# randyjhc/vit-colmap

Measured on AMD Instinct MI355X. Metric: images/sec extracted + pair-matches/sec (N×D brute-force NN), higher is better.
Workload: dtype bf16 (ViT) / u8+i32 (matcher); 1 GPU; configs[1]+configs[2]: DINOv2 ViT-S/14 extract of 50 640x480 images (512 keypoints, 384-D uint8 descriptors) then exhaustive mutual-NN + ratio matching of all pairs among the extracted images; images_total=50, images_rank0=50, num_keypoints=512, descriptor_dim=384, parallelism=images+pairs sharded x1

## Files before the change

### include/vitcolmap_hip.h

```cpp
#ifndef VITCOLMAP_HIP_H_
#define VITCOLMAP_HIP_H_

#include <stddef.h>
#include <stdint.h>

#ifdef __cplusplus
extern "C" {
#endif

#define VC_ABI_VERSION 1

#define VC_OK 0
#define VC_ERR_INVALID_ARG (-1)
#define VC_ERR_UNSUPPORTED (-2)
#define VC_ERR_LAUNCH (-3)
#define VC_ERR_WORKSPACE (-4)

#define VC_MAX_KEYPOINTS 2048
#define VC_MAX_DESC_DIM 1024
#define VC_MAX_NEIGHBOURS 64

typedef void* vc_stream_t;

int vc_abi_version(void);
// ... 83 lines not shown
#define VC_METHOD_HARRIS 0
#define VC_METHOD_DOG 1
#define VC_METHOD_COMBINED 2

int vc_structure_tensor(const void* tokens, int token_dtype, int n_images, int H, int W, int C,
                        float* st, vc_stream_t stream);

int vc_score_map(const float* st, int n_images, int H, int W, int method, float* score,
                 vc_stream_t stream);

int vc_select_keypoints(const float* score, int n_images, int H, int W, int target, int bin_size,
                        float nms_radius, int kmax, int32_t* out_yx, float* out_score,
                        int32_t* out_count, int32_t* dbg_cand_yx, float* dbg_cand_score,
                        int32_t* dbg_cand_count, vc_stream_t stream);

int vc_describe(const void* tokens, int token_dtype, int n_images, int H, int W, int C,
                const int32_t* yx, const int32_t* count, int kmax, const float* proj, int dd,
                int resized_w, int resized_h, int orig_w, int orig_h, float* out_kp,
                float* out_desc_f32, uint8_t* out_desc_u8, vc_stream_t stream);

#define VC_NORM_L2 0
#define VC_NORM_ROOTSIFT 1
int vc_describe_at(const void* tokens, int token_dtype, int n_images, int H, int W, int C, const float* keypoints_xy,
                   const int32_t* count, int kmax, const float* proj, int dd, int feat_w, int feat_h, int orig_w,
                   int orig_h, int normalisation, float* out_desc_f32, uint8_t* out_desc_u8, vc_stream_t stream);

int vc_quantize_u8(const float* in, uint8_t* out, size_t n, vc_stream_t stream);

size_t vc_heatmap_workspace_bytes(int n_images, int H, int W, int kmax);
int vc_heatmap_keypoints(const float* kp_map, const float* desc_map, long long desc_image_stride,
// ... 31 lines not shown
int vc_conv_taps_bf16(void* x, const void* weight, const void* bias, void* out, int batch, int height, int width, int c_in,
                      int n_out, int kh, int kw, int dy0, int dx0, int out_parity, int epilogue, vc_stream_t stream);

size_t vc_linear_xs_weight_bytes(int n_out, int k_in);
int vc_linear_xs_prepare(const float* weight, const float* bias_or_null, const float* ln_gamma_or_null,
                         const float* ln_beta_or_null, int n_out, int k_in, void* weight_tiled,
                         float* bias_folded, vc_stream_t stream);
int vc_linear_xs_bf16(const void* x, const void* weight_tiled, const float* bias_folded,
                      const void* residual_or_null, void* out, int rows, int n_out, int k_in, int epilogue,
                      int fuse_layernorm, float ln_eps, const void* gelu_table_or_null, vc_stream_t stream);
size_t vc_gelu_table_bytes(void);
int vc_gelu_table_bf16(void* table, vc_stream_t stream);

int vc_patch_embed_bf16(const void* patches, const void* weight, const void* bias, const void* pos_embed,
                        void* out, int n_images, int tokens, int n_out, int k_in, vc_stream_t stream);

size_t vc_mlp_weight_bytes(int n_hidden, int dim);
int vc_mlp_prepare(const float* w1, const float* b1_or_null, const float* ln_gamma_or_null,
                   const float* ln_beta_or_null, const float* w2, const float* b2_or_null, int n_hidden, int dim,
                   void* weights_tiled, float* b1_folded, float* b2_out, vc_stream_t stream);
int vc_mlp_bf16(void* x_inout, const void* weights_tiled, const float* b1_folded, const float* b2,
                const void* gelu_table, int rows, int n_hidden, int dim, float ln_eps, vc_stream_t stream);

#define VC_SIFT_MAX_RADIUS 64
#define VC_SIFT_NORM_L2 0
#define VC_SIFT_NORM_L1_ROOT 1

int vc_sift_grey(const uint8_t* images_bgr, int n_images, int h, int w, int out_h, int out_w, int upsample, float* out,
                 vc_stream_t stream);
int vc_sift_blur(const float* src, float* tmp, float* dst, int n_images, int h, int w, const float* taps, int radius,
// ... 31 lines not shown
```

### vit_colmap_amd/_lib.py

```python
import ctypes
import os
from ctypes import POINTER, c_char_p, c_double, c_float, c_int, c_int32, c_size_t, c_uint8, c_uint32, c_void_p

_HERE = os.path.dirname(os.path.abspath(__file__))
LIB_PATH = os.environ.get("VITCOLMAP_HIP_LIB") or os.path.join(_HERE, "libvitcolmap_hip.so")

VC_OK = 0
ABI_VERSION = 1
VC_MAX_KEYPOINTS = 2048
VC_MAX_DESC_DIM = 1024
VC_MAX_NEIGHBOURS = 64
VC_BA_MAX_CAMS = 512
VC_ERR_INVALID_ARG, VC_ERR_UNSUPPORTED, VC_ERR_LAUNCH, VC_ERR_WORKSPACE = -1, -2, -3, -4


class HipLibraryError(RuntimeError):
    pass


_u8p, _i32p, _u32p, _f32p = POINTER(c_uint8), POINTER(c_int32), POINTER(c_uint32), POINTER(ctypes.c_float)

SIGNATURES = {
    "vc_abi_version": (c_int, []),
    "vc_status_string": (c_char_p, [c_int]),
# ... 23 lines not shown
    "vc_p3p": (c_int, [c_void_p, c_void_p, c_void_p, c_int, c_void_p, c_int, c_void_p, c_void_p, c_void_p]),
    "vc_absolute_pose_score": (c_int, [c_void_p, c_void_p, c_void_p, c_int, c_void_p, c_int, c_float, c_void_p, c_void_p]),
    "vc_absolute_pose_inliers": (c_int, [c_void_p, c_void_p, c_void_p, c_int, c_void_p, c_float, c_void_p, c_void_p]),
    "vc_triangulate_tracks": (c_int, [c_void_p, c_void_p, c_void_p, c_int, c_void_p, c_int, c_void_p, c_double, c_double, c_void_p,
                                      c_void_p, c_void_p, c_void_p, c_void_p]),
    "vc_ba_linearize_points": (c_int, [c_void_p, c_int, c_void_p, c_void_p, c_int, c_void_p, c_void_p, c_void_p, c_int, c_double,
                                       c_void_p, c_void_p, c_void_p, c_void_p, c_void_p, c_void_p, c_void_p, c_void_p]),
    "vc_ba_reduce_cameras": (c_int, [c_int, c_void_p, c_int, c_void_p, c_void_p, c_int, c_void_p, c_void_p, c_void_p, c_double,
                                     c_void_p, c_void_p, c_void_p, c_void_p, c_void_p, c_void_p, c_void_p]),
    "vc_ba_step": (c_int, [c_void_p, c_int, c_void_p, c_int, c_void_p, c_void_p, c_int, c_void_p, c_void_p, c_void_p, c_void_p,
                           c_void_p, c_void_p, c_void_p, c_void_p, c_void_p]),
    "vc_structure_tensor": (c_int, [c_void_p, c_int, c_int, c_int, c_int, c_int, c_void_p, c_void_p]),
    "vc_score_map": (c_int, [c_void_p, c_int, c_int, c_int, c_int, c_void_p, c_void_p]),
    "vc_select_keypoints": (c_int, [c_void_p, c_int, c_int, c_int, c_int, c_int, c_float, c_int, c_void_p,
                                    c_void_p, c_void_p, c_void_p, c_void_p, c_void_p, c_void_p]),
    "vc_describe": (c_int, [c_void_p, c_int, c_int, c_int, c_int, c_int, c_void_p, c_void_p, c_int, c_void_p,
                            c_int, c_int, c_int, c_int, c_int, c_void_p, c_void_p, c_void_p, c_void_p]),
    "vc_describe_at": (c_int, [c_void_p, c_int, c_int, c_int, c_int, c_int, c_void_p, c_void_p, c_int, c_void_p, c_int, c_int,
                               c_int, c_int, c_int, c_int, c_void_p, c_void_p, c_void_p]),
    "vc_quantize_u8": (c_int, [c_void_p, c_void_p, c_size_t, c_void_p]),
    "vc_heatmap_workspace_bytes": (c_size_t, [c_int, c_int, c_int, c_int]),
    "vc_heatmap_keypoints": (c_int, [c_void_p, c_void_p, ctypes.c_longlong, ctypes.c_longlong, ctypes.c_longlong, c_int, c_int,
                                     c_int, c_int, c_int, c_float, c_int, c_float, c_float, c_float, c_float, c_void_p,
                                     c_void_p, c_void_p, c_void_p, c_void_p]),
    "vc_add_layernorm_bf16": (c_int, [c_void_p, c_void_p, c_void_p, c_void_p, c_float, c_int, c_int, c_void_p,
                                      c_void_p, c_void_p]),
    "vc_layernorm_drop_first_bf16": (c_int, [c_void_p, c_void_p, c_void_p, c_float, c_int, c_int, c_int, c_void_p, c_void_p]),
    "vc_attention_bf16": (c_int, [c_void_p, c_int, c_int, c_int, c_int, c_int, c_void_p, c_void_p]),
    "vc_linear_bf16": (c_int, [c_void_p, c_void_p, c_void_p, c_void_p, c_void_p, c_int, c_int, c_int, c_int, c_void_p]),
    "vc_conv_taps_bf16": (c_int, [c_void_p, c_void_p, c_void_p, c_void_p] + [c_int] * 11 + [c_void_p]),
    "vc_linear_xs_weight_bytes": (c_size_t, [c_int, c_int]),
    "vc_linear_xs_prepare": (c_int, [c_void_p, c_void_p, c_void_p, c_void_p, c_int, c_int, c_void_p, c_void_p, c_void_p]),
    "vc_linear_xs_bf16": (c_int, [c_void_p, c_void_p, c_void_p, c_void_p, c_void_p, c_int, c_int, c_int, c_int, c_int,
                                  c_float, c_void_p, c_void_p]),
    "vc_gelu_table_bytes": (c_size_t, []),
    "vc_gelu_table_bf16": (c_int, [c_void_p, c_void_p]),
    "vc_patch_embed_bf16": (c_int, [c_void_p, c_void_p, c_void_p, c_void_p, c_void_p, c_int, c_int, c_int, c_int, c_void_p]),
    "vc_mlp_weight_bytes": (c_size_t, [c_int, c_int]),
    "vc_mlp_prepare": (c_int, [c_void_p, c_void_p, c_void_p, c_void_p, c_void_p, c_void_p, c_int, c_int, c_void_p, c_void_p,
                               c_void_p, c_void_p]),
    "vc_mlp_bf16": (c_int, [c_void_p, c_void_p, c_void_p, c_void_p, c_void_p, c_int, c_int, c_int, c_float, c_void_p]),
    "vc_preprocess_u8": (c_int, [c_void_p, c_int, c_int, c_int, c_int, c_int, c_int, c_int, c_void_p, c_void_p,
                                 c_void_p]),
    "vc_sift_grey": (c_int, [c_void_p, c_int, c_int, c_int, c_int, c_int, c_int, c_void_p, c_void_p]),
    "vc_sift_blur": (c_int, [c_void_p, c_void_p, c_void_p, c_int, c_int, c_int, _f32p, c_int, c_void_p]),
    "vc_sift_downsample": (c_int, [c_void_p, c_int, c_int, c_int, c_void_p, c_void_p]),
    "vc_sift_dog": (c_int, [c_void_p, c_int, c_int, c_int, c_int, c_void_p, c_void_p]),
    "vc_sift_detect": (c_int, [c_void_p, c_int, c_int, c_int, c_int, c_float, c_float, c_int, c_void_p, c_int, c_void_p,
                               c_void_p, c_void_p]),
    "vc_sift_orient": (c_int, [c_void_p, c_int, c_int, c_int, c_int, c_void_p, c_void_p, c_int, c_int, c_int, c_void_p,
                               c_void_p, c_void_p]),
    "vc_sift_describe": (c_int, [c_void_p, c_int, c_int, c_int, c_int, c_void_p, c_void_p, c_int, c_void_p, c_void_p, c_int,
# ... 92 lines not shown
```

### vit_colmap_amd/csrc/gemm.hip

```cpp
#include <hip/hip_runtime.h>
#include <stdint.h>

#include "../../include/vitcolmap_hip.h"
#include "common.h"
#include "device.h"

namespace {

typedef __bf16 v8bf __attribute__((ext_vector_type(8)));
typedef __bf16 v4bf __attribute__((ext_vector_type(4)));
typedef __bf16 v2bf __attribute__((ext_vector_type(2)));
typedef float v16f __attribute__((ext_vector_type(16)));
typedef float v4f __attribute__((ext_vector_type(4)));
typedef float v2f __attribute__((ext_vector_type(2)));
typedef uint32_t v4u __attribute__((ext_vector_type(4)));
typedef uint32_t v2u __attribute__((ext_vector_type(2)));

__device__ __forceinline__ uint32_t pack_bf16x2(float lo, float hi) {
  const v2bf p = {(__bf16)lo, (__bf16)hi};
  return *(const uint32_t*)&p;
}
__device__ __forceinline__ v2f unpack_bf16x2(uint32_t u) { return (v2f){__uint_as_float(u << 16), __uint_as_float(u & 0xffff0000u)}; }

constexpr int BM = 128;
// ... 39 lines not shown
__device__ __forceinline__ float swiglu_f32(float a, float b) {
  const float e = __builtin_amdgcn_exp2f(a * -1.4426950408889634f);
  return a * __builtin_amdgcn_rcpf(1.0f + e) * b;
}

__device__ __forceinline__ uint32_t frag_off(int row0, int lane, int ks) {
  const int fr = lane & 15, ch = ks * 4 + (lane >> 4);
  return (uint32_t)(row0 + fr) * 128u + (uint32_t)((ch ^ (fr & 7)) << 4);
}

template <int EPI>
__global__ __launch_bounds__(256, 2) void gemm_kernel(const __bf16* __restrict__ X, const __bf16* __restrict__ W,
                                                      const __bf16* __restrict__ bias,
                                                      const __bf16* __restrict__ res, __bf16* __restrict__ out,
                                                      int M, int N, int K, int n_tiles_n, int n_tiles,
                                                      int group) {
  __shared__ __attribute__((aligned(1024))) uint8_t lds[2][kStage];
  const int tid = threadIdx.x, lane = tid & 63;
  const int wave = __builtin_amdgcn_readfirstlane(tid >> 6);
  const int wm = wave & 1, wn = wave >> 1;

  const int tile = vc::xcd_tile(blockIdx.x, n_tiles);
  const int tm = tile / n_tiles_n, tn = tile - tm * n_tiles_n;
  const int m0 = tm * BM, n0 = tn * BN;
  const int H = N >> 1, j0 = tn * (BN / 2);

  const uint32_t lds0 = vc::lds_addr(&lds[0][0]);
  const int prow = lane >> 3, pchunk = (lane & 7) ^ prow;
  const __bf16* xsrc[4];
  const __bf16* wsrc[4];
#pragma unroll
// ... 86 lines not shown
#pragma unroll
        for (int j = 0; j < 4; ++j) v[j] = acc[a][b][j] + (float)bv[j];
        if (EPI == EPI_GELU) {
#pragma unroll
          for (int j = 0; j < 4; ++j) v[j] = gelu_erf(v[j]);
        }
        if (EPI == EPI_RESIDUAL || EPI == EPI_PATCH) {
          const v4bf rv = *(const v4bf*)(res + ro);
#pragma unroll
          for (int j = 0; j < 4; ++j) v[j] += (float)rv[j];
        }
        v4bf ov;
#pragma unroll
        for (int j = 0; j < 4; ++j) ov[j] = (__bf16)v[j];
        *(v4bf*)(out + o) = ov;
      }
    }
  }
}


constexpr int G2M = 256, G2N = 256;
constexpr int kUnit2 = 128 * 128;
constexpr int kBuf2 = 4 * kUnit2;
constexpr int G256_LDS = 2 * kBuf2;
constexpr int kAhead2 = 6;

template <int EPI, bool CONV>
__global__ __launch_bounds__(512, 2) void gemm256_kernel(const __bf16* __restrict__ X, const __bf16* __restrict__ W,
                                                         const __bf16* __restrict__ bias, const __bf16* __restrict__ res,
// ... 887 lines not shown
    static vc::PerDeviceOnce configured;
    if (int st = vc::allow_dynamic_lds(configured, G256_LDS, gemm256_kernel<EPI_BIAS, false>, gemm256_kernel<EPI_GELU, false>,
                                       gemm256_kernel<EPI_RESIDUAL, false>, gemm256_kernel<EPI_SWIGLU, false>))
      return st;
    const dim3 grid(persistent_grid(nt, cus)), block(512);
    return vc::dispatch<EPI_BIAS, EPI_GELU, EPI_RESIDUAL, EPI_SWIGLU>(epilogue, [&](auto epi) {
      hipLaunchKernelGGL((gemm256_kernel<epi, false>), grid, block, (size_t)G256_LDS, s, px, pw, pb, pr, po, rows, n_out, k_in,
                         tiles_n, (int)nt, 0, 0, 0, 1, 0, 0, -1);
      return vc::check_launch();
    });
  }
  const int tiles_m = (rows + BM - 1) / BM, tiles_n = n_out / BN;
  const long long nt = (long long)tiles_m * tiles_n;
  if (nt > 0x7fffffffLL) return VC_ERR_UNSUPPORTED;
  return vc::dispatch<EPI_BIAS, EPI_GELU, EPI_RESIDUAL, EPI_SWIGLU>(epilogue, [&](auto epi) {
    hipLaunchKernelGGL(gemm_kernel<epi>, dim3((unsigned)nt), dim3(256), 0, s, px, pw, pb, pr, po, rows, n_out, k_in, tiles_n, (int)nt, 1);
    return vc::check_launch();
  });
}


int vc_conv_taps_bf16(void* x, const void* weight, const void* bias, void* out, int batch, int height, int width, int c_in,
                      int n_out, int kh, int kw, int dy0, int dx0, int out_parity, int epilogue, vc_stream_t stream) {
  if (!x || !weight || !bias || !out || batch < 0 || height <= 0 || width <= 0 || c_in <= 0 || n_out <= 0) return VC_ERR_INVALID_ARG;
  if (epilogue != EPI_BIAS && epilogue != EPI_GELU) return VC_ERR_INVALID_ARG;
  if (kh <= 0 || kw <= 0 || kh * kw > 16 || dy0 < -8 || dy0 > 8 || dx0 < -8 || dx0 > 8) return VC_ERR_INVALID_ARG;
  if (out_parity < -1 || out_parity > 3) return VC_ERR_INVALID_ARG;
  if (n_out % G2N != 0 || c_in % BK != 0) return VC_ERR_UNSUPPORTED;
  if (!aligned16(x, weight, bias, out)) return VC_ERR_INVALID_ARG;
  const long long rows = (long long)batch * height * width;
  if (rows == 0) return VC_OK;
// ... 72 lines not shown
                         ln_eps, gt);
      return vc::check_launch();
    };
    return vc::dispatch<EPI_BIAS, EPI_GELU, EPI_RESIDUAL>(epilogue, [&](auto epi) {
      return vc::dispatch<true, false>(fuse_layernorm != 0, [&](auto ln) {
        if constexpr (epi == EPI_GELU) {
          if (use_gt) return launch(epi, ln, std::true_type{});
        }
        return launch(epi, ln, std::false_type{});
      });
    });
  });
}


int vc_patch_embed_bf16(const void* patches, const void* weight, const void* bias, const void* pos_embed, void* out,
                        int n_images, int tokens, int n_out, int k_in, vc_stream_t stream) {
  if (!patches || !weight || !bias || !pos_embed || !out || n_images < 0 || tokens <= 0 || n_out <= 0 || k_in <= 0)
    return VC_ERR_INVALID_ARG;
  if (n_out % BN != 0 || k_in % BK != 0) return VC_ERR_UNSUPPORTED;
  if (!aligned16(patches, weight, bias, pos_embed, out)) return VC_ERR_INVALID_ARG;
  if (n_images == 0) return VC_OK;
  const long long rows = (long long)n_images * tokens;
  const long long nt = ((rows + BM - 1) / BM) * (n_out / BN);
  if (rows > 0x7fffffffLL || nt > 0x7fffffffLL) return VC_ERR_UNSUPPORTED;
  hipLaunchKernelGGL(gemm_kernel<EPI_PATCH>, dim3((unsigned)nt), dim3(256), 0, (hipStream_t)stream, (const __bf16*)patches,
                     (const __bf16*)weight, (const __bf16*)bias, (const __bf16*)pos_embed, (__bf16*)out, (int)rows, n_out,
                     k_in, n_out / BN, (int)nt, tokens);
  return vc::check_launch();
}


size_t vc_mlp_weight_bytes(int n_hidden, int dim) {
  if (dim != XK || n_hidden <= 0 || n_hidden % 32 != 0 || n_hidden > mlp_lds().max_hidden()) return 0;
  return (size_t)(n_hidden / 32) * MStage;
}

int vc_mlp_prepare(const float* w1, const float* b1_or_null, const float* ln_gamma_or_null, const float* ln_beta_or_null,
                   const float* w2, const float* b2_or_null, int n_hidden, int dim, void* weights_tiled, float* b1_folded,
                   float* b2_out, vc_stream_t stream) {
  if (!w1 || !w2 || !weights_tiled || !b1_folded || !b2_out) return VC_ERR_INVALID_ARG;
  if (vc_mlp_weight_bytes(n_hidden, dim) == 0) return VC_ERR_UNSUPPORTED;
  if ((ln_gamma_or_null == nullptr) != (ln_beta_or_null == nullptr)) return VC_ERR_INVALID_ARG;
  hipLaunchKernelGGL(mlp_prepare_kernel, dim3((n_hidden + XK + 3) / 4), dim3(256), 0, (hipStream_t)stream, w1, b1_or_null,
// ... 22 lines not shown
```

### vit_colmap_amd/csrc/select.hip

```cpp
#include <hip/hip_runtime.h>
#include <stdint.h>

#include "../../include/vitcolmap_hip.h"
#include "common.h"
#include "device.h"

namespace {

constexpr int kMaxCells = 16384;
constexpr int kMaxCandidates = 4096;
constexpr int kSelThreads = 512;

template <typename T>
__device__ inline float load_token(const T* p, int i);
template <>
__device__ inline float load_token<float>(const float* p, int i) { return p[i]; }
template <>
__device__ inline float load_token<uint16_t>(const uint16_t* p, int i) { return vc::bf16_to_f32(p[i]); }

__device__ inline float wave_sum(float v) {
#pragma unroll
  for (int o = 32; o > 0; o >>= 1) v += __shfl_xor(v, o);
  return v;
}
// ... 111 lines not shown
  if (hi > 0.f)
    for (int i = threadIdx.x; i < cells; i += blockDim.x) m[i] = m[i] / hi;
  __syncthreads();
}

__device__ inline void minmax_eps(float* m, int cells, float* scratch) {
  float lo = INFINITY, hi = -INFINITY;
  for (int i = threadIdx.x; i < cells; i += blockDim.x) { lo = fminf(lo, m[i]); hi = fmaxf(hi, m[i]); }
  lo = block_reduce(lo, false, scratch);
  hi = block_reduce(hi, true, scratch);
  const float den = (hi - lo) + 1e-8f;
  for (int i = threadIdx.x; i < cells; i += blockDim.x) m[i] = (m[i] - lo) / den;
  __syncthreads();
}

__global__ __launch_bounds__(kSelThreads) void score_kernel(const float* __restrict__ st, int H, int W, int method,
                                                            Taps g3, Taps g7, Taps g11, float* __restrict__ score) {
  extern __shared__ __attribute__((aligned(16))) float lds[];
  const int cells = H * W;
  float* a = lds;
  float* b = lds + cells;
  float* scratch = lds + 2 * cells;
  const int img = blockIdx.x;
  const float* ixx = st + (size_t)img * 4 * cells;
  const float* iyy = ixx + cells;
  const float* ixy = iyy + cells;
  const float* avg = ixy + cells;

  if (method == 0 || method == 2) {
    for (int i = threadIdx.x; i < cells; i += blockDim.x) {
      const int y = i / W, x = i - y * W;
      const float sxx = smooth(ixx, H, W, y, x, g3);
      const float syy = smooth(iyy, H, W, y, x, g3);
      const float sxy = smooth(ixy, H, W, y, x, g3);
      const float det = sxx * syy - sxy * sxy;
      const float tr = sxx + syy;
      const float corner = det - 0.04f * (tr * tr);
      const float edge = sqrtf(sxx + syy);
      a[i] = 0.7f * corner + 0.3f * edge;
    }
    __syncthreads();
    minmax01(a, cells, scratch);
  }
  if (method == 1 || method == 2) {
    float* o = method == 1 ? a : b;
    for (int i = threadIdx.x; i < cells; i += blockDim.x) {
      const int y = i / W, x = i - y * W;
      o[i] = fabsf(smooth(avg, H, W, y, x, g7) - smooth(avg, H, W, y, x, g11));
    }
    __syncthreads();
    minmax01(o, cells, scratch);
  }
  if (method == 2) {
    minmax_eps(a, cells, scratch);
    minmax_eps(b, cells, scratch);
    for (int i = threadIdx.x; i < cells; i += blockDim.x) a[i] = 0.5f * a[i] + 0.5f * b[i];
    __syncthreads();
  }
  for (int i = threadIdx.x; i < cells; i += blockDim.x) score[(size_t)img * cells + i] = a[i];
}

__device__ inline bool before(float sa, int pa, float sb, int pb) { return sa > sb || (sa == sb && pa < pb); }

__global__ __launch_bounds__(kSelThreads) void select_kernel(const float* __restrict__ score_g, int H, int W,
                                                             int target, int bin, int nms_reach, int nms_d2_max, int kmax,
                                                             int32_t* __restrict__ out_yx,
                                                             float* __restrict__ out_score,
                                                             int32_t* __restrict__ out_count,
                                                             int32_t* __restrict__ dbg_cand_yx,
                                                             float* __restrict__ dbg_cand_score,
                                                             int32_t* __restrict__ dbg_cand_count) {
  extern __shared__ __attribute__((aligned(16))) float lds[];
  const int cells = H * W;
  const int tid = threadIdx.x, nt = blockDim.x;
  const int img = blockIdx.x;
  float* score = lds;
  int* cand_cell = (int*)(lds + cells);
  float* cand_score = (float*)(cand_cell + kMaxCandidates);
  int* tmp_cell = (int*)(cand_score + kMaxCandidates);
  float* tmp_score = (float*)(tmp_cell + kMaxCandidates);
  int* state = (int*)(tmp_score + kMaxCandidates);
  int* cell_rank = state + kMaxCandidates;
  __shared__ int s_wave_tot[kSelThreads / 64];

  for (int i = tid; i < cells; i += nt) score[i] = score_g[(size_t)img * cells + i];
  __syncthreads();

  const int nbh = max(1, H / bin), nbw = max(1, W / bin);
  const int per_bin = max(1, target / (nbh * nbw));
  const int bh = min(bin, H), bw = min(bin, W), n = bh * bw;
  const int k = min(per_bin, n);
  const int K_bins = nbh * nbw * k;
  for (int idx = tid; idx < nbh * nbw * n; idx += nt) {
    const int b = idx / n, e = idx - b * n;
    const int bi = b / nbw, bj = b - bi * nbw;
    const int y0 = bi * bin, x0 = bj * bin;
    const int ey = e / bw, ex = e - ey * bw;
    const float s = score[(y0 + ey) * W + x0 + ex];
    int rank = 0;
    for (int oy = 0; oy < bh; ++oy)
      for (int ox = 0; ox < bw; ++ox)
// ... 97 lines not shown
        out_yx[((size_t)img * kmax + pos) * 2 + 0] = cell / W;
        out_yx[((size_t)img * kmax + pos) * 2 + 1] = cell % W;
        out_score[(size_t)img * kmax + pos] = tmp_score[r];
      }
    }
    base += tot;
    __syncthreads();
  }
  const int total = min(base, kmax);
  for (int p = total + tid; p < kmax; p += nt) {
    out_yx[((size_t)img * kmax + p) * 2 + 0] = 0;
    out_yx[((size_t)img * kmax + p) * 2 + 1] = 0;
    out_score[(size_t)img * kmax + p] = 0.f;
  }
  if (tid == 0) out_count[img] = total;
}

template <typename T>
__global__ __launch_bounds__(256) void describe_kernel(const T* __restrict__ tokens, int H, int W, int C,
                                                       const int32_t* __restrict__ yx,
                                                       const int32_t* __restrict__ count, int kmax,
                                                       const float* __restrict__ proj, int dd, float sx1,
                                                       float sx2, float sy1, float sy2,
                                                       float* __restrict__ out_kp, float* __restrict__ out_f32,
                                                       uint8_t* __restrict__ out_u8,
                                                       const float* __restrict__ kp_in, int rootsift) {
  extern __shared__ __attribute__((aligned(16))) float lds[];
  const int lane = threadIdx.x & 63, wave = threadIdx.x >> 6;
  const int img = blockIdx.y;
  const int m = blockIdx.x * 4 + wave;
// ... 84 lines not shown

Taps make_taps(int k, float sigma) {
  Taps t;
  t.k = k;
  float sum = 0.f;
  for (int i = 0; i < k; ++i) {
    const float x = (float)i - (float)(k / 2);
    t.w[i] = expf(-(x * x) / (float)(2.0 * (double)sigma * (double)sigma));
    sum += t.w[i];
  }
  for (int i = 0; i < k; ++i) t.w[i] = t.w[i] / sum;
  for (int i = k; i < 11; ++i) t.w[i] = 0.f;
  return t;
}

}

extern "C" {

int vc_structure_tensor(const void* tokens, int token_dtype, int n_images, int H, int W, int C, float* st,
                        vc_stream_t stream) {
  if (!tokens || !st || n_images < 0 || H <= 0 || W <= 0 || C <= 0) return VC_ERR_INVALID_ARG;
  if (token_dtype != VC_DTYPE_F32 && token_dtype != VC_DTYPE_BF16) return VC_ERR_INVALID_ARG;
  if (n_images == 0) return VC_OK;
  const dim3 grid((H * W + 3) / 4, n_images);
  const bool vec_ok = C % 8 == 0 && ((uintptr_t)tokens) % 16 == 0;
  if (token_dtype == VC_DTYPE_F32)
    hipLaunchKernelGGL(structure_tensor_kernel<float>, grid, dim3(256), 0, (hipStream_t)stream,
                       (const float*)tokens, H, W, C, st, vec_ok);
  else
// ... 9 lines not shown
  if (n_images == 0) return VC_OK;
  const size_t smem = ((size_t)2 * H * W + 32) * sizeof(float);
  static vc::PerDeviceOnce configured;
  if (int st = vc::allow_dynamic_lds(configured, (int)((2 * kMaxCells + 32) * sizeof(float)), score_kernel)) return st;
  const Taps g3 = make_taps(3, 1.0f), g7 = make_taps(7, 1.0f), g11 = make_taps(11, 1.6f);
  hipLaunchKernelGGL(score_kernel, dim3(n_images), dim3(kSelThreads), smem, (hipStream_t)stream, st, H, W,
                     method, g3, g7, g11, score);
  return vc::check_launch();
}

int vc_select_keypoints(const float* score, int n_images, int H, int W, int target, int bin_size,
                        float nms_radius, int kmax, int32_t* out_yx, float* out_score, int32_t* out_count,
                        int32_t* dbg_cand_yx, float* dbg_cand_score, int32_t* dbg_cand_count,
                        vc_stream_t stream) {
  if (!score || !out_yx || !out_score || !out_count) return VC_ERR_INVALID_ARG;
  if (n_images < 0 || H <= 0 || W <= 0 || target <= 0 || bin_size <= 0 || kmax <= 0) return VC_ERR_INVALID_ARG;
  if (!(nms_radius >= 0.f) || nms_radius > 8.f) return VC_ERR_UNSUPPORTED;
  if ((dbg_cand_count != nullptr) != (dbg_cand_yx != nullptr) || (dbg_cand_count != nullptr) != (dbg_cand_score != nullptr))
    return VC_ERR_INVALID_ARG;
  const long cells = (long)H * W;
  const int nb = (H / bin_size > 0 ? H / bin_size : 1) * (W / bin_size > 0 ? W / bin_size : 1);
  const long cand = (long)nb * (target / nb > 0 ? target / nb : 1);
  if (cells > kMaxCells || cand > kMaxCandidates || target > kMaxCandidates) return VC_ERR_UNSUPPORTED;
  if (kmax < (cand < target ? cand : target)) return VC_ERR_INVALID_ARG;
  if (n_images == 0) return VC_OK;
  const size_t smem = (size_t)cells * 4 * 2 + (size_t)kMaxCandidates * 4 * 5;
  constexpr int kDynMax = 160 * 1024 - 1024;
  if (smem > (size_t)kDynMax) return VC_ERR_UNSUPPORTED;
  static vc::PerDeviceOnce configured;
  if (int st = vc::allow_dynamic_lds(configured, kDynMax, select_kernel)) return st;
  int nms_d2_max = 0;
  while (nms_d2_max < 2 * 8 * 8 && sqrtf((float)(nms_d2_max + 1)) < nms_radius) ++nms_d2_max;
  const int nms_reach = (int)sqrtf((float)nms_d2_max);
  hipLaunchKernelGGL(select_kernel, dim3(n_images), dim3(kSelThreads), smem, (hipStream_t)stream, score, H, W,
                     target, bin_size, nms_reach, nms_d2_max, kmax, out_yx, out_score, out_count, dbg_cand_yx,
                     dbg_cand_score, dbg_cand_count);
  return vc::check_launch();
}

int vc_describe(const void* tokens, int token_dtype, int n_images, int H, int W, int C, const int32_t* yx,
                const int32_t* count, int kmax, const float* proj, int dd, int resized_w, int resized_h,
                int orig_w, int orig_h, float* out_kp, float* out_desc_f32, uint8_t* out_desc_u8,
                vc_stream_t stream) {
  if (!tokens || !yx || !count || !out_kp || !out_desc_u8) return VC_ERR_INVALID_ARG;
  if (n_images < 0 || H <= 1 || W <= 1 || C <= 0 || kmax <= 0) return VC_ERR_INVALID_ARG;
  if (token_dtype != VC_DTYPE_F32 && token_dtype != VC_DTYPE_BF16) return VC_ERR_INVALID_ARG;
  if (proj && dd <= 0) return VC_ERR_INVALID_ARG;
  if (resized_w <= 0 || resized_h <= 0 || orig_w <= 0 || orig_h <= 0) return VC_ERR_INVALID_ARG;
  if (n_images == 0) return VC_OK;
  const int out_dim = proj ? dd : C;
  const size_t smem = (size_t)4 * (C + out_dim) * sizeof(float);
// ... 51 lines not shown
```

### vit_colmap_amd/features/hip_select.py

```python
import torch

from .. import _lib

METHODS = {"harris": 0, "dog": 1, "combined": 2}


def _dtype_code(t):
    if t.dtype == torch.float32:
        return 0
    if t.dtype == torch.bfloat16:
        return 1
    raise _lib.HipLibraryError(f"tokens must be float32 or bfloat16, got {t.dtype}")


def _check_tokens(tokens, H, W):
    if not tokens.is_cuda:
        raise _lib.HipLibraryError("tokens must live on the GPU (no CPU fallback)")
    assert tokens.dim() == 3 and tokens.is_contiguous() and tokens.shape[1] == H * W, tokens.shape


def structure_tensor(tokens: torch.Tensor, H: int, W: int) -> torch.Tensor:
    _check_tokens(tokens, H, W)
    lib = _lib.load()
    B, _, C = tokens.shape
# ... 22 lines not shown
    if kmax is None:
        kmax = target
    dev = score.device
    yx = torch.empty((B, kmax, 2), dtype=torch.int32, device=dev)
    sc = torch.empty((B, kmax), dtype=torch.float32, device=dev)
    cnt = torch.empty((B,), dtype=torch.int32, device=dev)
    dbg = (None, None, None)
    if debug_candidates:
        dbg = (torch.zeros_like(yx), torch.zeros_like(sc), torch.zeros_like(cnt))
    _lib.check(lib.vc_select_keypoints(_lib.ptr(score), B, H, W, target, bin_size, nms_radius, kmax, _lib.ptr(yx),
                                       _lib.ptr(sc), _lib.ptr(cnt), _lib.ptr(dbg[0]), _lib.ptr(dbg[1]),
                                       _lib.ptr(dbg[2]), _lib.stream_ptr()), "vc_select_keypoints")
    return (yx, sc, cnt, dbg) if debug_candidates else (yx, sc, cnt)


def describe(tokens: torch.Tensor, H: int, W: int, yx: torch.Tensor, count: torch.Tensor, resized_wh,
             original_wh, projection=None, want_f32: bool = False):
    _check_tokens(tokens, H, W)
    lib = _lib.load()
    B, _, C = tokens.shape
    kmax = yx.shape[1]
    dd = 0
    if projection is not None:
        assert projection.is_cuda and projection.dtype == torch.float32 and projection.is_contiguous()
        assert projection.shape[0] == C
        dd = projection.shape[1]
    D = dd if projection is not None else C
    dev = tokens.device
    kp = torch.empty((B, kmax, 2), dtype=torch.float32, device=dev)
    u8 = torch.empty((B, kmax, D), dtype=torch.uint8, device=dev)
# ... 25 lines not shown
               "vc_describe_at")
    return (u8, f32) if want_f32 else u8


def quantize_u8(x: torch.Tensor) -> torch.Tensor:
    assert x.is_cuda and x.dtype == torch.float32 and x.is_contiguous()
    lib = _lib.load()
    out = torch.empty(x.shape, dtype=torch.uint8, device=x.device)
    _lib.check(lib.vc_quantize_u8(_lib.ptr(x), _lib.ptr(out), x.numel(), _lib.stream_ptr()), "vc_quantize_u8")
    return out


def dense_to_sparse(tokens, H, W, original_wh, resized_wh, num_keypoints, method="harris", projection=None,
                    bin_size=16, nms_radius=1.5, want_f32=False):
    st = structure_tensor(tokens, H, W)
    score = score_map(st, H, W, method)
    yx, sc, cnt = select_keypoints(score, num_keypoints, bin_size, nms_radius)
    out = describe(tokens, H, W, yx, cnt, resized_wh, original_wh, projection, want_f32)
    res = dict(keypoints=out[0], desc_u8=out[1], count=cnt, yx=yx, scores=sc, score=score)
    if want_f32:
        res["desc_f32"] = out[2]
    return res


def heatmap_workspace_bytes(n_images: int, H: int, W: int, kmax: int) -> int:
    return _lib.load().vc_heatmap_workspace_bytes(n_images, H, W, kmax)


def heatmap_keypoints(kp_map: torch.Tensor, desc_map: torch.Tensor, num_keypoints: int, score_threshold: float,
                      nms_radius: int, original_wh, resized_wh):
    if not (kp_map.is_cuda and desc_map.is_cuda):
        raise _lib.HipLibraryError("head outputs must live on the GPU (no CPU fallback)")
# ... 22 lines not shown
```

### vit_colmap_amd/vit/dinov2.py

```python
import math
from dataclasses import dataclass

import torch
import torch.nn as nn
import torch.nn.functional as F

PATCH = 14


@dataclass(frozen=True)
class Arch:
    dim: int
    depth: int
    heads: int
    ffn: str = "mlp"
    registers: int = 0
    img_size: int = 518


DINOV2_ARCHS = {
    "dinov2_vits14": Arch(384, 12, 6),
    "dinov2_vitb14": Arch(768, 12, 12),
    "dinov2_vitl14": Arch(1024, 24, 16),
    "dinov2_vitg14": Arch(1536, 40, 24, ffn="swiglu"),
# ... 186 lines not shown
        return bool(getattr(self, "_hip", None)) and self.register_tokens is None and not self.training

    def forward_patch_tokens(self, patches: torch.Tensor, hp: int, wp: int) -> torch.Tensor:
        B = patches.shape[0]
        if patches.shape[-1] == 640:
            if not (patches.is_cuda and patches.dtype == torch.bfloat16 and self.register_tokens is None and not self.training):
                raise ValueError("padded patches are only accepted by the bf16 GPU path")
            if getattr(self, "_hip", None) is None:
                self.prepare_hip()
            if not self._hip:
                raise ValueError("padded patches need a model that prepare_hip() covers")
            from . import hip_ops as ops

            pos, cls_row = self._padded_pos(hp, wp, patches.device)
            x = torch.empty((B, 1 + hp * wp, self.arch.dim), dtype=torch.bfloat16, device=patches.device)
            ops.patch_embed(patches, self._pe_w, self.patch_embed.proj.bias, pos, x)
            x[:, 0] = cls_row
            return self._blocks_hip(x)
        if patches.is_cuda and patches.dtype == torch.bfloat16 and getattr(self, "_hip", None) and not self.training:
            from . import hip_ops as ops

            x = ops.linear(F.pad(patches, (0, self._pe_w.shape[1] - patches.shape[-1])), self._pe_w, self.patch_embed.proj.bias)
        else:
            x = self.patch_embed.forward_patches(patches)
        x = torch.cat([self.cls_token.expand(B, -1, -1), x], dim=1) + self.interpolated_pos_embed(hp, wp)
        if self.register_tokens is not None:
            x = torch.cat([x[:, :1], self.register_tokens.expand(B, -1, -1), x[:, 1:]], dim=1)
        if x.is_cuda and x.dtype == torch.bfloat16 and all(b.folded for b in self.blocks) and not self.training:
            x = self._blocks_fused(x.contiguous())
        else:
            for blk in self.blocks:
                x = blk(x)
# ... 190 lines not shown
```

### vit_colmap_amd/vit/hip_ops.py

```python
import torch

from .. import _lib


def add_layernorm(x: torch.Tensor, residual, weight: torch.Tensor, bias: torch.Tensor, eps: float,
                  want_sum: bool = True):
    assert x.is_cuda and x.dtype == torch.bfloat16 and x.is_contiguous()
    lib = _lib.load()
    C = x.shape[-1]
    rows = x.numel() // C
    y = torch.empty_like(x)
    s = torch.empty_like(x) if (residual is not None and want_sum) else None
    if residual is not None:
        assert residual.shape == x.shape and residual.dtype == x.dtype and residual.is_contiguous()
    _lib.check(lib.vc_add_layernorm_bf16(_lib.ptr(x), _lib.ptr(residual), _lib.ptr(weight), _lib.ptr(bias), eps, rows, C,
                                         _lib.ptr(s), _lib.ptr(y), _lib.stream_ptr()), "vc_add_layernorm_bf16")
    return s, y


def layernorm_drop_first(x: torch.Tensor, weight: torch.Tensor, bias: torch.Tensor, eps: float, out=None) -> torch.Tensor:
    assert x.is_cuda and x.dtype == torch.bfloat16 and x.is_contiguous() and x.dim() == 3
    B, N, C = x.shape
    y = torch.empty((B, N - 1, C), dtype=torch.bfloat16, device=x.device) if out is None else out
    assert y.shape == (B, N - 1, C) and y.dtype == torch.bfloat16 and y.is_contiguous()
# ... 101 lines not shown
        if out is None:
            out = torch.empty(x.shape[:-1] + (self.n,), dtype=torch.bfloat16, device=x.device)
        if residual is not None:
            assert residual.shape == out.shape and residual.dtype == torch.bfloat16 and residual.is_contiguous()
        lib = _lib.load()
        _lib.check(lib.vc_linear_xs_bf16(_lib.ptr(x), _lib.ptr(self.wp), _lib.ptr(self.bias), _lib.ptr(residual),
                                         _lib.ptr(out), rows, self.n, self.k, epilogue, int(self.ln), self.eps,
                                         _lib.ptr(gelu_table), _lib.stream_ptr()), "vc_linear_xs_bf16")
        return out


PATCH_K_PADDED = 640


def patch_embed(patches: torch.Tensor, weight_padded: torch.Tensor, bias: torch.Tensor, pos_embed: torch.Tensor,
                out: torch.Tensor) -> torch.Tensor:
    B, T, K = patches.shape
    C = weight_padded.shape[0]
    assert patches.is_cuda and patches.dtype == torch.bfloat16 and patches.is_contiguous() and K == weight_padded.shape[1]
    assert weight_padded.is_contiguous() and bias.is_contiguous() and pos_embed.is_contiguous() and out.is_contiguous()
    assert pos_embed.shape[-2:] == (T + 1, C) and out.shape == (B, T + 1, C) and out.dtype == torch.bfloat16
    lib = _lib.load()
    _lib.check(lib.vc_patch_embed_bf16(_lib.ptr(patches), _lib.ptr(weight_padded), _lib.ptr(bias), _lib.ptr(pos_embed),
                                       _lib.ptr(out), B, T, C, K, _lib.stream_ptr()), "vc_patch_embed_bf16")
    return out


_GELU_TABLES = {}


def gelu_table(device) -> torch.Tensor:
    key = torch.device(device)
    if key not in _GELU_TABLES:
        lib = _lib.load()
        t = torch.empty(lib.vc_gelu_table_bytes(), dtype=torch.uint8, device=key)
        _lib.check(lib.vc_gelu_table_bf16(_lib.ptr(t), _lib.stream_ptr()), "vc_gelu_table_bf16")
        _GELU_TABLES[key] = t
    return _GELU_TABLES[key]

# ... 28 lines not shown
```

Before: 7841 images/s.

## Fuse score map with keypoint selection and CLS row write into patch embed

```diff
diff --git a/include/vitcolmap_hip.h b/include/vitcolmap_hip.h
--- a/include/vitcolmap_hip.h
+++ b/include/vitcolmap_hip.h
@@ -121,6 +121,11 @@
                         int32_t* out_count, int32_t* dbg_cand_yx, float* dbg_cand_score,
                         int32_t* dbg_cand_count, vc_stream_t stream);
 
+int vc_score_select_fits(int H, int W, int method);
+int vc_score_select(const float* st, int n_images, int H, int W, int method, int target, int bin_size,
+                    float nms_radius, int kmax, float* score, int32_t* out_yx, float* out_score,
+                    int32_t* out_count, vc_stream_t stream);
+
 int vc_describe(const void* tokens, int token_dtype, int n_images, int H, int W, int C,
                 const int32_t* yx, const int32_t* count, int kmax, const float* proj, int dd,
                 int resized_w, int resized_h, int orig_w, int orig_h, float* out_kp,
@@ -182,6 +187,9 @@
 
 int vc_patch_embed_bf16(const void* patches, const void* weight, const void* bias, const void* pos_embed,
                         void* out, int n_images, int tokens, int n_out, int k_in, vc_stream_t stream);
+int vc_patch_embed_cls_bf16(const void* patches, const void* weight, const void* bias, const void* pos_embed,
+                            const void* cls_row_or_null, void* out, int n_images, int tokens, int n_out, int k_in,
+                            vc_stream_t stream);
 
 size_t vc_mlp_weight_bytes(int n_hidden, int dim);
 int vc_mlp_prepare(const float* w1, const float* b1_or_null, const float* ln_gamma_or_null,
diff --git a/vit_colmap_amd/_lib.py b/vit_colmap_amd/_lib.py
--- a/vit_colmap_amd/_lib.py
+++ b/vit_colmap_amd/_lib.py
@@ -61,6 +61,9 @@
     "vc_score_map": (c_int, [c_void_p, c_int, c_int, c_int, c_int, c_void_p, c_void_p]),
     "vc_select_keypoints": (c_int, [c_void_p, c_int, c_int, c_int, c_int, c_int, c_float, c_int, c_void_p,
                                     c_void_p, c_void_p, c_void_p, c_void_p, c_void_p, c_void_p]),
+    "vc_score_select_fits": (c_int, [c_int, c_int, c_int]),
+    "vc_score_select": (c_int, [c_void_p, c_int, c_int, c_int, c_int, c_int, c_int, c_float, c_int, c_void_p, c_void_p,
+                                c_void_p, c_void_p, c_void_p]),
     "vc_describe": (c_int, [c_void_p, c_int, c_int, c_int, c_int, c_int, c_void_p, c_void_p, c_int, c_void_p,
                             c_int, c_int, c_int, c_int, c_int, c_void_p, c_void_p, c_void_p, c_void_p]),
     "vc_describe_at": (c_int, [c_void_p, c_int, c_int, c_int, c_int, c_int, c_void_p, c_void_p, c_int, c_void_p, c_int, c_int,
@@ -83,6 +86,8 @@
     "vc_gelu_table_bytes": (c_size_t, []),
     "vc_gelu_table_bf16": (c_int, [c_void_p, c_void_p]),
     "vc_patch_embed_bf16": (c_int, [c_void_p, c_void_p, c_void_p, c_void_p, c_void_p, c_int, c_int, c_int, c_int, c_void_p]),
+    "vc_patch_embed_cls_bf16": (c_int, [c_void_p, c_void_p, c_void_p, c_void_p, c_void_p, c_void_p, c_int, c_int, c_int, c_int,
+                                        c_void_p]),
     "vc_mlp_weight_bytes": (c_size_t, [c_int, c_int]),
     "vc_mlp_prepare": (c_int, [c_void_p, c_void_p, c_void_p, c_void_p, c_void_p, c_void_p, c_int, c_int, c_void_p, c_void_p,
                                c_void_p, c_void_p]),
diff --git a/vit_colmap_amd/csrc/gemm.hip b/vit_colmap_amd/csrc/gemm.hip
--- a/vit_colmap_amd/csrc/gemm.hip
+++ b/vit_colmap_amd/csrc/gemm.hip
@@ -77,7 +77,7 @@
                                                       const __bf16* __restrict__ bias,
                                                       const __bf16* __restrict__ res, __bf16* __restrict__ out,
                                                       int M, int N, int K, int n_tiles_n, int n_tiles,
-                                                      int group) {
+                                                      int group, const __bf16* __restrict__ cls_row) {
   __shared__ __attribute__((aligned(1024))) uint8_t lds[2][kStage];
   const int tid = threadIdx.x, lane = tid & 63;
   const int wave = __builtin_amdgcn_readfirstlane(tid >> 6);
@@ -194,6 +194,9 @@
 #pragma unroll
         for (int j = 0; j < 4; ++j) ov[j] = (__bf16)v[j];
         *(v4bf*)(out + o) = ov;
+        if (EPI == EPI_PATCH) {
+          if (cls_row && ro == (size_t)N + n) *(v4bf*)(out + o - N) = *(const v4bf*)(cls_row + n);
+        }
       }
     }
   }
@@ -1111,7 +1114,8 @@
   const long long nt = (long long)tiles_m * tiles_n;
   if (nt > 0x7fffffffLL) return VC_ERR_UNSUPPORTED;
   return vc::dispatch<EPI_BIAS, EPI_GELU, EPI_RESIDUAL, EPI_SWIGLU>(epilogue, [&](auto epi) {
-    hipLaunchKernelGGL(gemm_kernel<epi>, dim3((unsigned)nt), dim3(256), 0, s, px, pw, pb, pr, po, rows, n_out, k_in, tiles_n, (int)nt, 1);
+    hipLaunchKernelGGL(gemm_kernel<epi>, dim3((unsigned)nt), dim3(256), 0, s, px, pw, pb, pr, po, rows, n_out, k_in, tiles_n, (int)nt, 1,
+                       (const __bf16*)nullptr);
     return vc::check_launch();
   });
 }
@@ -1214,20 +1218,26 @@
 }
 
 
-int vc_patch_embed_bf16(const void* patches, const void* weight, const void* bias, const void* pos_embed, void* out,
-                        int n_images, int tokens, int n_out, int k_in, vc_stream_t stream) {
+int vc_patch_embed_cls_bf16(const void* patches, const void* weight, const void* bias, const void* pos_embed,
+                            const void* cls_row_or_null, void* out, int n_images, int tokens, int n_out, int k_in,
+                            vc_stream_t stream) {
   if (!patches || !weight || !bias || !pos_embed || !out || n_images < 0 || tokens <= 0 || n_out <= 0 || k_in <= 0)
     return VC_ERR_INVALID_ARG;
   if (n_out % BN != 0 || k_in % BK != 0) return VC_ERR_UNSUPPORTED;
-  if (!aligned16(patches, weight, bias, pos_embed, out)) return VC_ERR_INVALID_ARG;
+  if (!aligned16(patches, weight, bias, pos_embed, cls_row_or_null, out)) return VC_ERR_INVALID_ARG;
   if (n_images == 0) return VC_OK;
   const long long rows = (long long)n_images * tokens;
   const long long nt = ((rows + BM - 1) / BM) * (n_out / BN);
   if (rows > 0x7fffffffLL || nt > 0x7fffffffLL) return VC_ERR_UNSUPPORTED;
   hipLaunchKernelGGL(gemm_kernel<EPI_PATCH>, dim3((unsigned)nt), dim3(256), 0, (hipStream_t)stream, (const __bf16*)patches,
                      (const __bf16*)weight, (const __bf16*)bias, (const __bf16*)pos_embed, (__bf16*)out, (int)rows, n_out,
-                     k_in, n_out / BN, (int)nt, tokens);
+                     k_in, n_out / BN, (int)nt, tokens, (const __bf16*)cls_row_or_null);
   return vc::check_launch();
+}
+
+int vc_patch_embed_bf16(const void* patches, const void* weight, const void* bias, const void* pos_embed, void* out,
+                        int n_images, int tokens, int n_out, int k_in, vc_stream_t stream) {
+  return vc_patch_embed_cls_bf16(patches, weight, bias, pos_embed, nullptr, out, n_images, tokens, n_out, k_in, stream);
 }
 
 
diff --git a/vit_colmap_amd/csrc/select.hip b/vit_colmap_amd/csrc/select.hip
--- a/vit_colmap_amd/csrc/select.hip
+++ b/vit_colmap_amd/csrc/select.hip
@@ -149,19 +149,10 @@
   __syncthreads();
 }
 
-__global__ __launch_bounds__(kSelThreads) void score_kernel(const float* __restrict__ st, int H, int W, int method,
-                                                            Taps g3, Taps g7, Taps g11, float* __restrict__ score) {
-  extern __shared__ __attribute__((aligned(16))) float lds[];
+__device__ inline void score_body(const float* ixx, const float* iyy, const float* ixy, const float* avg, int H, int W,
+                                  int method, const Taps& g3, const Taps& g7, const Taps& g11, float* a, float* b,
+                                  float* scratch) {
   const int cells = H * W;
-  float* a = lds;
-  float* b = lds + cells;
-  float* scratch = lds + 2 * cells;
-  const int img = blockIdx.x;
-  const float* ixx = st + (size_t)img * 4 * cells;
-  const float* iyy = ixx + cells;
-  const float* ixy = iyy + cells;
-  const float* avg = ixy + cells;
-
   if (method == 0 || method == 2) {
     for (int i = threadIdx.x; i < cells; i += blockDim.x) {
       const int y = i / W, x = i - y * W;
@@ -192,23 +183,31 @@
     for (int i = threadIdx.x; i < cells; i += blockDim.x) a[i] = 0.5f * a[i] + 0.5f * b[i];
     __syncthreads();
   }
-  for (int i = threadIdx.x; i < cells; i += blockDim.x) score[(size_t)img * cells + i] = a[i];
-}
-
-__device__ inline bool before(float sa, int pa, float sb, int pb) { return sa > sb || (sa == sb && pa < pb); }
-
-__global__ __launch_bounds__(kSelThreads) void select_kernel(const float* __restrict__ score_g, int H, int W,
-                                                             int target, int bin, int nms_reach, int nms_d2_max, int kmax,
-                                                             int32_t* __restrict__ out_yx,
-                                                             float* __restrict__ out_score,
-                                                             int32_t* __restrict__ out_count,
-                                                             int32_t* __restrict__ dbg_cand_yx,
-                                                             float* __restrict__ dbg_cand_score,
-                                                             int32_t* __restrict__ dbg_cand_count) {
+}
+
+__global__ __launch_bounds__(kSelThreads) void score_kernel(const float* __restrict__ st, int H, int W, int method,
+                                                            Taps g3, Taps g7, Taps g11, float* __restrict__ score) {
   extern __shared__ __attribute__((aligned(16))) float lds[];
   const int cells = H * W;
+  float* a = lds;
+  float* b = lds + cells;
+  float* scratch = lds + 2 * cells;
+  const int img = blockIdx.x;
+  const float* ixx = st + (size_t)img * 4 * cells;
+  score_body(ixx, ixx + cells, ixx + 2 * cells, ixx + 3 * cells, H, W, method, g3, g7, g11, a, b, scratch);
+  for (int i = threadIdx.x; i < cells; i += blockDim.x) score[(size_t)img * cells + i] = a[i];
+}
+
+__device__ inline bool before(float sa, int pa, float sb, int pb) { return sa > sb || (sa == sb && pa < pb); }
+
+constexpr size_t select_lds_floats(size_t cells) { return 2 * cells + 5 * (size_t)kMaxCandidates; }
+
+__device__ inline void select_body(float* lds, int img, int H, int W, int target, int bin, int nms_reach, int nms_d2_max,
+                                   int kmax, int32_t* __restrict__ out_yx, float* __restrict__ out_score,
+                                   int32_t* __restrict__ out_count, int32_t* __restrict__ dbg_cand_yx,
+                                   float* __restrict__ dbg_cand_score, int32_t* __restrict__ dbg_cand_count) {
+  const int cells = H * W;
   const int tid = threadIdx.x, nt = blockDim.x;
-  const int img = blockIdx.x;
   float* score = lds;
   int* cand_cell = (int*)(lds + cells);
   float* cand_score = (float*)(cand_cell + kMaxCandidates);
@@ -217,9 +216,6 @@
   int* state = (int*)(tmp_score + kMaxCandidates);
   int* cell_rank = state + kMaxCandidates;
   __shared__ int s_wave_tot[kSelThreads / 64];
-
-  for (int i = tid; i < cells; i += nt) score[i] = score_g[(size_t)img * cells + i];
-  __syncthreads();
 
   const int nbh = max(1, H / bin), nbw = max(1, W / bin);
   const int per_bin = max(1, target / (nbh * nbw));
@@ -347,6 +343,61 @@
     out_score[(size_t)img * kmax + p] = 0.f;
   }
   if (tid == 0) out_count[img] = total;
+}
+
+__global__ __launch_bounds__(kSelThreads) void select_kernel(const float* __restrict__ score_g, int H, int W,
+                                                             int target, int bin, int nms_reach, int nms_d2_max, int kmax,
+                                                             int32_t* __restrict__ out_yx,
+                                                             float* __restrict__ out_score,
+                                                             int32_t* __restrict__ out_count,
+                                                             int32_t* __restrict__ dbg_cand_yx,
+                                                             float* __restrict__ dbg_cand_score,
+                                                             int32_t* __restrict__ dbg_cand_count) {
+  extern __shared__ __attribute__((aligned(16))) float lds[];
+  const int cells = H * W;
+  const int img = blockIdx.x;
+  for (int i = threadIdx.x; i < cells; i += blockDim.x) lds[i] = score_g[(size_t)img * cells + i];
+  __syncthreads();
+  select_body(lds, img, H, W, target, bin, nms_reach, nms_d2_max, kmax, out_yx, out_score, out_count, dbg_cand_yx,
+              dbg_cand_score, dbg_cand_count);
+}
+
+constexpr int kScoreScratch = 32;
+constexpr int kSelLdsMax = 160 * 1024 - 1024;
+struct ScoreSelectPlan {
+  int maps;
+  size_t floats;
+  constexpr ScoreSelectPlan(size_t cells, int method)
+      : maps(method == 0 ? 3 : method == 1 ? 1 : 4), floats(0) {
+    const size_t score_phase = cells * (size_t)(1 + maps + (method == 2 ? 1 : 0)) + kScoreScratch;
+    floats = score_phase > select_lds_floats(cells) ? score_phase : select_lds_floats(cells);
+  }
+  constexpr bool fits() const { return floats * sizeof(float) <= (size_t)kSelLdsMax; }
+};
+
+__global__ __launch_bounds__(kSelThreads) void score_select_kernel(const float* __restrict__ st, int H, int W, int method,
+                                                                   Taps g3, Taps g7, Taps g11, int target, int bin,
+                                                                   int nms_reach, int nms_d2_max, int kmax,
+                                                                   float* __restrict__ score_out,
+                                                                   int32_t* __restrict__ out_yx,
+                                                                   float* __restrict__ out_score,
+                                                                   int32_t* __restrict__ out_count) {
+  extern __shared__ __attribute__((aligned(16))) float lds[];
+  const int cells = H * W;
+  const int img = blockIdx.x;
+  const ScoreSelectPlan plan((size_t)cells, method);
+  float* a = lds;
+  float* maps = lds + cells;
+  float* b = maps + (size_t)plan.maps * cells;
+  float* scratch = b + (method == 2 ? cells : 0);
+  const float* src = st + ((size_t)img * 4 + (method == 1 ? 3 : 0)) * cells;
+  for (int i = threadIdx.x; i < plan.maps * cells; i += blockDim.x) maps[i] = src[i];
+  __syncthreads();
+  const float* avg = method == 1 ? maps : maps + 3 * (size_t)cells;
+  score_body(maps, maps + cells, maps + 2 * (size_t)cells, avg, H, W, method, g3, g7, g11, a, b, scratch);
+  for (int i = threadIdx.x; i < cells; i += blockDim.x) score_out[(size_t)img * cells + i] = a[i];
+  select_body(lds, img, H, W, target, bin, nms_reach, nms_d2_max, kmax, out_yx, out_score, out_count, nullptr, nullptr,
+              nullptr);
 }
 
 template <typename T>
@@ -461,6 +512,25 @@
   return t;
 }
 
+int check_selection(int n_images, int H, int W, int target, int bin_size, float nms_radius, int kmax) {
+  if (n_images < 0 || H <= 0 || W <= 0 || target <= 0 || bin_size <= 0 || kmax <= 0) return VC_ERR_INVALID_ARG;
+  if (!(nms_radius >= 0.f) || nms_radius > 8.f) return VC_ERR_UNSUPPORTED;
+  const long cells = (long)H * W;
+  const int nb = (H / bin_size > 0 ? H / bin_size : 1) * (W / bin_size > 0 ? W / bin_size : 1);
+  const long cand = (long)nb * (target / nb > 0 ? target / nb : 1);
+  if (cells > kMaxCells || cand > kMaxCandidates || target > kMaxCandidates) return VC_ERR_UNSUPPORTED;
+  if (kmax < (cand < target ? cand : target)) return VC_ERR_INVALID_ARG;
+  return VC_OK;
+}
+
+struct NmsBound {
+  int d2_max = 0, reach = 0;
+  explicit NmsBound(float nms_radius) {
+    while (d2_max < 2 * 8 * 8 && sqrtf((float)(d2_max + 1)) < nms_radius) ++d2_max;
+    reach = (int)sqrtf((float)d2_max);
+  }
+};
+
 }
 
 extern "C" {
@@ -500,27 +570,41 @@
                         int32_t* dbg_cand_yx, float* dbg_cand_score, int32_t* dbg_cand_count,
                         vc_stream_t stream) {
   if (!score || !out_yx || !out_score || !out_count) return VC_ERR_INVALID_ARG;
-  if (n_images < 0 || H <= 0 || W <= 0 || target <= 0 || bin_size <= 0 || kmax <= 0) return VC_ERR_INVALID_ARG;
-  if (!(nms_radius >= 0.f) || nms_radius > 8.f) return VC_ERR_UNSUPPORTED;
   if ((dbg_cand_count != nullptr) != (dbg_cand_yx != nullptr) || (dbg_cand_count != nullptr) != (dbg_cand_score != nullptr))
     return VC_ERR_INVALID_ARG;
-  const long cells = (long)H * W;
-  const int nb = (H / bin_size > 0 ? H / bin_size : 1) * (W / bin_size > 0 ? W / bin_size : 1);
-  const long cand = (long)nb * (target / nb > 0 ? target / nb : 1);
-  if (cells > kMaxCells || cand > kMaxCandidates || target > kMaxCandidates) return VC_ERR_UNSUPPORTED;
-  if (kmax < (cand < target ? cand : target)) return VC_ERR_INVALID_ARG;
+  if (int st = check_selection(n_images, H, W, target, bin_size, nms_radius, kmax)) return st;
   if (n_images == 0) return VC_OK;
-  const size_t smem = (size_t)cells * 4 * 2 + (size_t)kMaxCandidates * 4 * 5;
-  constexpr int kDynMax = 160 * 1024 - 1024;
-  if (smem > (size_t)kDynMax) return VC_ERR_UNSUPPORTED;
+  const size_t smem = select_lds_floats((size_t)H * W) * sizeof(float);
+  if (smem > (size_t)kSelLdsMax) return VC_ERR_UNSUPPORTED;
   static vc::PerDeviceOnce configured;
-  if (int st = vc::allow_dynamic_lds(configured, kDynMax, select_kernel)) return st;
-  int nms_d2_max = 0;
-  while (nms_d2_max < 2 * 8 * 8 && sqrtf((float)(nms_d2_max + 1)) < nms_radius) ++nms_d2_max;
-  const int nms_reach = (int)sqrtf((float)nms_d2_max);
+  if (int st = vc::allow_dynamic_lds(configured, kSelLdsMax, select_kernel)) return st;
+  const NmsBound nms(nms_radius);
   hipLaunchKernelGGL(select_kernel, dim3(n_images), dim3(kSelThreads), smem, (hipStream_t)stream, score, H, W,
-                     target, bin_size, nms_reach, nms_d2_max, kmax, out_yx, out_score, out_count, dbg_cand_yx,
+                     target, bin_size, nms.reach, nms.d2_max, kmax, out_yx, out_score, out_count, dbg_cand_yx,
                      dbg_cand_score, dbg_cand_count);
+  return vc::check_launch();
+}
+
+int vc_score_select_fits(int H, int W, int method) {
+  if (H <= 0 || W <= 0 || method < 0 || method > 2 || (long)H * W > kMaxCells) return 0;
+  return ScoreSelectPlan((size_t)H * W, method).fits() ? 1 : 0;
+}
+
+int vc_score_select(const float* st, int n_images, int H, int W, int method, int target, int bin_size, float nms_radius,
+                    int kmax, float* score, int32_t* out_yx, float* out_score, int32_t* out_count, vc_stream_t stream) {
+  if (!st || !score || !out_yx || !out_score || !out_count) return VC_ERR_INVALID_ARG;
+  if (method < 0 || method > 2) return VC_ERR_INVALID_ARG;
+  if (int status = check_selection(n_images, H, W, target, bin_size, nms_radius, kmax)) return status;
+  const ScoreSelectPlan plan((size_t)H * W, method);
+  if (!plan.fits()) return VC_ERR_UNSUPPORTED;
+  if (n_images == 0) return VC_OK;
+  static vc::PerDeviceOnce configured;
+  if (int status = vc::allow_dynamic_lds(configured, kSelLdsMax, score_select_kernel)) return status;
+  const Taps g3 = make_taps(3, 1.0f), g7 = make_taps(7, 1.0f), g11 = make_taps(11, 1.6f);
+  const NmsBound nms(nms_radius);
+  hipLaunchKernelGGL(score_select_kernel, dim3(n_images), dim3(kSelThreads), plan.floats * sizeof(float), (hipStream_t)stream,
+                     st, H, W, method, g3, g7, g11, target, bin_size, nms.reach, nms.d2_max, kmax, score, out_yx, out_score,
+                     out_count);
   return vc::check_launch();
 }
 
diff --git a/vit_colmap_amd/features/hip_select.py b/vit_colmap_amd/features/hip_select.py
--- a/vit_colmap_amd/features/hip_select.py
+++ b/vit_colmap_amd/features/hip_select.py
@@ -60,6 +60,31 @@
     return (yx, sc, cnt, dbg) if debug_candidates else (yx, sc, cnt)
 
 
+def score_select_fits(H: int, W: int, method: str = "harris") -> bool:
+    if method not in METHODS:
+        raise ValueError(f"Unknown detection method: {method}")
+    return bool(_lib.load().vc_score_select_fits(H, W, METHODS[method]))
+
+
+def score_select(st: torch.Tensor, H: int, W: int, method: str, target: int, bin_size: int = 16, nms_radius: float = 1.5,
+                 kmax=None):
+    if method not in METHODS:
+        raise ValueError(f"Unknown detection method: {method}")
+    assert st.is_cuda and st.dtype == torch.float32 and st.is_contiguous() and st.shape[1:] == (4, H * W)
+    lib = _lib.load()
+    B = st.shape[0]
+    if kmax is None:
+        kmax = target
+    dev = st.device
+    score = torch.empty((B, H, W), dtype=torch.float32, device=dev)
+    yx = torch.empty((B, kmax, 2), dtype=torch.int32, device=dev)
+    sc = torch.empty((B, kmax), dtype=torch.float32, device=dev)
+    cnt = torch.empty((B,), dtype=torch.int32, device=dev)
+    _lib.check(lib.vc_score_select(_lib.ptr(st), B, H, W, METHODS[method], target, bin_size, nms_radius, kmax, _lib.ptr(score),
+                                   _lib.ptr(yx), _lib.ptr(sc), _lib.ptr(cnt), _lib.stream_ptr()), "vc_score_select")
+    return score, yx, sc, cnt
+
+
 def describe(tokens: torch.Tensor, H: int, W: int, yx: torch.Tensor, count: torch.Tensor, resized_wh,
              original_wh, projection=None, want_f32: bool = False):
     _check_tokens(tokens, H, W)
@@ -115,8 +140,11 @@
 def dense_to_sparse(tokens, H, W, original_wh, resized_wh, num_keypoints, method="harris", projection=None,
                     bin_size=16, nms_radius=1.5, want_f32=False):
     st = structure_tensor(tokens, H, W)
-    score = score_map(st, H, W, method)
-    yx, sc, cnt = select_keypoints(score, num_keypoints, bin_size, nms_radius)
+    if score_select_fits(H, W, method):
+        score, yx, sc, cnt = score_select(st, H, W, method, num_keypoints, bin_size, nms_radius)
+    else:
+        score = score_map(st, H, W, method)
+        yx, sc, cnt = select_keypoints(score, num_keypoints, bin_size, nms_radius)
     out = describe(tokens, H, W, yx, cnt, resized_wh, original_wh, projection, want_f32)
     res = dict(keypoints=out[0], desc_u8=out[1], count=cnt, yx=yx, scores=sc, score=score)
     if want_f32:
diff --git a/vit_colmap_amd/vit/dinov2.py b/vit_colmap_amd/vit/dinov2.py
--- a/vit_colmap_amd/vit/dinov2.py
+++ b/vit_colmap_amd/vit/dinov2.py
@@ -224,8 +224,7 @@
 
             pos, cls_row = self._padded_pos(hp, wp, patches.device)
             x = torch.empty((B, 1 + hp * wp, self.arch.dim), dtype=torch.bfloat16, device=patches.device)
-            ops.patch_embed(patches, self._pe_w, self.patch_embed.proj.bias, pos, x)
-            x[:, 0] = cls_row
+            ops.patch_embed(patches, self._pe_w, self.patch_embed.proj.bias, pos, x, cls_row)
             return self._blocks_hip(x)
         if patches.is_cuda and patches.dtype == torch.bfloat16 and getattr(self, "_hip", None) and not self.training:
             from . import hip_ops as ops
diff --git a/vit_colmap_amd/vit/hip_ops.py b/vit_colmap_amd/vit/hip_ops.py
--- a/vit_colmap_amd/vit/hip_ops.py
+++ b/vit_colmap_amd/vit/hip_ops.py
@@ -139,15 +139,18 @@
 
 
 def patch_embed(patches: torch.Tensor, weight_padded: torch.Tensor, bias: torch.Tensor, pos_embed: torch.Tensor,
-                out: torch.Tensor) -> torch.Tensor:
+                out: torch.Tensor, cls_row=None) -> torch.Tensor:
     B, T, K = patches.shape
     C = weight_padded.shape[0]
     assert patches.is_cuda and patches.dtype == torch.bfloat16 and patches.is_contiguous() and K == weight_padded.shape[1]
     assert weight_padded.is_contiguous() and bias.is_contiguous() and pos_embed.is_contiguous() and out.is_contiguous()
     assert pos_embed.shape[-2:] == (T + 1, C) and out.shape == (B, T + 1, C) and out.dtype == torch.bfloat16
+    if cls_row is not None:
+        assert cls_row.is_cuda and cls_row.dtype == torch.bfloat16 and cls_row.is_contiguous() and cls_row.shape == (C,)
     lib = _lib.load()
-    _lib.check(lib.vc_patch_embed_bf16(_lib.ptr(patches), _lib.ptr(weight_padded), _lib.ptr(bias), _lib.ptr(pos_embed),
-                                       _lib.ptr(out), B, T, C, K, _lib.stream_ptr()), "vc_patch_embed_bf16")
+    _lib.check(lib.vc_patch_embed_cls_bf16(_lib.ptr(patches), _lib.ptr(weight_padded), _lib.ptr(bias), _lib.ptr(pos_embed),
+                                           _lib.ptr(cls_row), _lib.ptr(out), B, T, C, K, _lib.stream_ptr()),
+               "vc_patch_embed_cls_bf16")
     return out
 
 
```

Measured after the change: 7842 images/s, median of 2. Within noise of the previous version (+0.0%).
